# sigma0-dev/polymath

Hardware: AMD Instinct MI355X
Metric: prove_constraints_per_sec (higher is better)
Workload: dtype u32; 1 GPU; 2^20-100-constraint synthetic R1CS (random A*B=C gates), bls12_381, n=2^21, transcript=merlin; msm_pairs_per_proof=29359963, parallelism=one GPU

## Files before the change

### polymath_amd/csrc/radix.cuh

```cuda
#pragma once
#include <stdint.h>

#if defined(__HIPCC__)
#define PM_RADIX_HD __host__ __device__ __forceinline__
#else
#define PM_RADIX_HD inline
#endif

namespace pm {

constexpr uint32_t RADIX_NO_DIGIT = 0xFFFFFFFFu;

template <class P>
constexpr bool radix_top_fits(unsigned m, unsigned W, unsigned a) {
    static_assert(P::N == 8, "256-bit scalars");
    if (m == 0 || m > 7 || W == 0 || a == 0 || a > 28) return false;
    uint32_t p[8] = {1, 0, 0, 0, 0, 0, 0, 0};
    for (unsigned j = 0; j < W; ++j) {
        uint64_t c = 0;
        for (int i = 0; i < 8; ++i) {
            c += (uint64_t)p[i] * m;
            p[i] = (uint32_t)c;
            c >>= 32;
        }
        if (c) return true;
    }
    const unsigned s = a * W - 1;
    if (s >= 256) return true;
    uint32_t t[8] = {0, 0, 0, 0, 0, 0, 0, 0};
    for (int i = 0; i < 8; ++i) {
        const unsigned src = (unsigned)i + s / 32;
        if (src >= 8) break;
        const uint32_t lo = P::MOD[src] - (src == 0 ? 1u : 0u);
        const uint32_t hi = src + 1 < 8 ? P::MOD[src + 1] : 0u;
        t[i] = s % 32 ? (lo >> (s % 32)) | (hi << (32 - s % 32)) : lo;
    }
    for (int i = 7; i >= 0; --i)
        if (t[i] != p[i]) return t[i] < p[i];
    return false;
}
template <class P>
constexpr unsigned radix_min_shift(unsigned m, unsigned W) {
    for (unsigned a = 1; a <= 28; ++a)
        if (radix_top_fits<P>(m, W, a)) return a;
    return 0;
}

template <unsigned W, unsigned A, unsigned w>
PM_RADIX_HD void radix5_recode_from(uint32_t (&k)[8], uint32_t &carry, uint32_t (&out)[W]) {
    if constexpr (w < W) {
        constexpr int bits = 256 - (int)(w * (A + 2));
        constexpr int nl = bits > 0 ? (bits + 31) / 32 : 0;
        constexpr int nl2 = bits > (int)A ? (bits - (int)A + 31) / 32 : 0;
        const uint32_t low = nl ? k[0] & ((1u << A) - 1) : 0u;
#pragma unroll
        for (int i = 0; i < nl; ++i) k[i] = (k[i] >> A) | (i + 1 < nl ? k[i + 1] << (32 - A) : 0u);
        uint32_t rem = 0;
#pragma unroll
        for (int i = nl2 - 1; i >= 0; --i) {
            const uint32_t x = k[i];
            const uint32_t t = (uint32_t)(((uint64_t)x * 0xCCCCCCCDu) >> 34);
            const uint32_t s = rem + (x - 5u * t);
            const uint32_t e = s >= 5u ? 1u : 0u;
            k[i] = rem * 0x33333333u + t + e;
            rem = s - 5u * e;
        }
        constexpr uint32_t full = 5u << A, half = 5u << (A - 1);
        const uint32_t d = (rem << A) + low + carry;
        const bool over = d > half;
        const uint32_t m = over ? full - d : d;
        carry = over ? 1u : 0u;
        out[w] = m ? ((m - 1) << 1) | carry : RADIX_NO_DIGIT;
        radix5_recode_from<W, A, w + 1>(k, carry, out);
    }
}

template <unsigned W, unsigned A>
PM_RADIX_HD uint32_t radix5_recode(const uint32_t (&scalar)[8], uint32_t (&out)[W]) {
    static_assert(A >= 1 && A <= 28, "R / 2 + 1 and (bucket << 1 | sign) fit 32 bits");
    uint32_t k[8];
#pragma unroll
    for (int i = 0; i < 8; ++i) k[i] = scalar[i];
    uint32_t carry = 0;
    radix5_recode_from<W, A, 0>(k, carry, out);
    return carry;
}

}
```

Before: 18.40 million constraints/s.

## Recode radix-5 scalar digits by top-down division with constant reciprocals

Replaces the per-window multi-limb shift-and-divide-by-5 loop with a top-down scheme. It extracts the bits above all windows, then divides by 5^w for each window using a precomputed reciprocal and a one-step correction. Signed-digit recoding becomes a separate cheap pass. This targets the quadratic per-scalar cost of repeated 256-bit divisions during MSM scalar recoding. In exchange it tightens the allowed parameter range (A<=24, A*W in [192,256)).

New measurement: 18.37 million constraints/s. About the same (-0.1%).

```diff
diff --git a/polymath_amd/csrc/radix.cuh b/polymath_amd/csrc/radix.cuh
--- a/polymath_amd/csrc/radix.cuh
+++ b/polymath_amd/csrc/radix.cuh
@@ -46,43 +46,69 @@
     return 0;
 }
 
+constexpr uint64_t radix_pow5(unsigned w) { uint64_t p = 1; for (unsigned i = 0; i < w; ++i) p *= 5; return p; }
+constexpr unsigned radix_bitlen(uint64_t v) { unsigned n = 0; for (; v; v >>= 1) ++n; return n; }
+
+template <unsigned POS, unsigned N>
+PM_RADIX_HD uint32_t radix_bits(const uint32_t (&k)[8]) {
+    constexpr unsigned i = POS / 32, s = POS % 32;
+    if constexpr (i >= 8) {
+        return 0u;
+    } else {
+        uint32_t v = k[i] >> s;
+        if constexpr (s + N > 32 && i + 1 < 8) v |= k[i + 1] << (32 - s);
+        if constexpr (N < 32) v &= (1u << N) - 1u;
+        return v;
+    }
+}
+
 template <unsigned W, unsigned A, unsigned w>
-PM_RADIX_HD void radix5_recode_from(uint32_t (&k)[8], uint32_t &carry, uint32_t (&out)[W]) {
-    if constexpr (w < W) {
-        constexpr int bits = 256 - (int)(w * (A + 2));
-        constexpr int nl = bits > 0 ? (bits + 31) / 32 : 0;
-        constexpr int nl2 = bits > (int)A ? (bits - (int)A + 31) / 32 : 0;
-        const uint32_t low = nl ? k[0] & ((1u << A) - 1) : 0u;
-#pragma unroll
-        for (int i = 0; i < nl; ++i) k[i] = (k[i] >> A) | (i + 1 < nl ? k[i + 1] << (32 - A) : 0u);
-        uint32_t rem = 0;
-#pragma unroll
-        for (int i = nl2 - 1; i >= 0; --i) {
-            const uint32_t x = k[i];
-            const uint32_t t = (uint32_t)(((uint64_t)x * 0xCCCCCCCDu) >> 34);
-            const uint32_t s = rem + (x - 5u * t);
-            const uint32_t e = s >= 5u ? 1u : 0u;
-            k[i] = rem * 0x33333333u + t + e;
-            rem = s - 5u * e;
+PM_RADIX_HD void radix5_divide_from(const uint32_t (&k)[8], uint64_t rho, uint32_t (&out)[W]) {
+    const uint32_t c = radix_bits<A * w, A>(k);
+    if constexpr (w == 0) {
+        out[0] = ((uint32_t)rho << A) | c;
+    } else {
+        constexpr uint64_t D = radix_pow5(w);
+        constexpr unsigned L = radix_bitlen(D), T = L > 4 ? L - 4 : 0;
+        static_assert(32 + T <= 63, "the reciprocal's numerator fits 64 bits: 5^w < 2^35");
+        constexpr uint32_t M = (uint32_t)(((uint64_t)1 << (32 + T)) / D);
+        constexpr bool rho32 = w + 1 == W ? A * W >= 224 : radix_pow5(w + 1) <= ((uint64_t)1 << 32);
+        if constexpr (rho32 && D < ((uint64_t)1 << 31)) {
+            const uint32_t r = (uint32_t)rho;
+            uint32_t xh;
+            if constexpr (T >= A) xh = r >> (T - A); else xh = (r << (A - T)) | (c >> T);
+            const uint32_t q = (uint32_t)(((uint64_t)xh * M) >> 32);
+            const uint32_t rem = ((r << A) | c) - q * (uint32_t)D;
+            const bool more = rem >= (uint32_t)D;
+            out[w] = q + (more ? 1u : 0u);
+            radix5_divide_from<W, A, w - 1>(k, rem - (more ? (uint32_t)D : 0u), out);
+        } else {
+            const uint64_t x = (rho << A) | c;
+            const uint32_t q = (uint32_t)(((uint64_t)(uint32_t)(x >> T) * M) >> 32);
+            const uint64_t rem = x - (uint64_t)q * D;
+            const bool more = rem >= D;
+            out[w] = q + (more ? 1u : 0u);
+            radix5_divide_from<W, A, w - 1>(k, rem - (more ? D : 0u), out);
         }
-        constexpr uint32_t full = 5u << A, half = 5u << (A - 1);
-        const uint32_t d = (rem << A) + low + carry;
-        const bool over = d > half;
-        const uint32_t m = over ? full - d : d;
-        carry = over ? 1u : 0u;
-        out[w] = m ? ((m - 1) << 1) | carry : RADIX_NO_DIGIT;
-        radix5_recode_from<W, A, w + 1>(k, carry, out);
     }
 }
 
 template <unsigned W, unsigned A>
 PM_RADIX_HD uint32_t radix5_recode(const uint32_t (&scalar)[8], uint32_t (&out)[W]) {
-    static_assert(A >= 1 && A <= 28, "R / 2 + 1 and (bucket << 1 | sign) fit 32 bits");
-    uint32_t k[8];
+    static_assert(A >= 1 && A <= 24, "R / 2 + 1 and (bucket << 1 | sign) fit 32 bits; the quotient estimate's bound (radix5_divide_from)");
+    static_assert(W >= 1 && W <= 16 && A * W >= 192 && A * W < 256, "5^w < 2^35, and the bits above the windows fit 64");
+    const uint64_t top = radix_bits<A * W, 32>(scalar) | ((uint64_t)radix_bits<A * W + 32, 32>(scalar) << 32);
+    radix5_divide_from<W, A, W - 1>(scalar, top, out);
+    constexpr uint32_t full = 5u << A, half = 5u << (A - 1);
+    uint32_t carry = 0;
 #pragma unroll
-    for (int i = 0; i < 8; ++i) k[i] = scalar[i];
-    uint32_t carry = 0;
-    radix5_recode_from<W, A, 0>(k, carry, out);
+    for (unsigned w = 0; w < W; ++w) {
+        const uint32_t d = out[w] + carry;
+        const bool over = d > half;
+        const uint32_t m = over ? full - d : d;
+        carry = over ? 1u : 0u;
+        out[w] = m ? ((m - 1) << 1) | carry : RADIX_NO_DIGIT;
+    }
     return carry;
 }
 
```
